# mvenouziou/Boosted_DETR

Hardware: AMD Instinct MI355X
Metric: images/sec training step (fwd+matcher+loss+bwd), 640x640 N=100 (higher is better)
Workload: dtype f32 (conv/GEMM products as 3 split-f16 [fwd] / split-bf16 [grad] MFMA products, f32 accumulate)

## Files before the change

### boosted_detr_amd/csrc/p16.hip

```cpp
#include "p16.h"

namespace {

__global__ __launch_bounds__(256) void p16_pack_kernel(const float* __restrict__ x, int64_t n8, void* __restrict__ f16_out, void* __restrict__ bf16_out,
                                                       int* __restrict__ overflow_flag, float f16_scale) {
    for (int64_t i = (int64_t)blockIdx.x * blockDim.x + threadIdx.x; i < n8; i += (int64_t)gridDim.x * blockDim.x) {
        const f32x4 a = reinterpret_cast<const f32x4*>(x)[2 * i], b = reinterpret_cast<const f32x4*>(x)[2 * i + 1];
        const float v[8] = {a[0], a[1], a[2], a[3], b[0], b[1], b[2], b[3]};
        if (f16_out) {
            const float vs[8] = {v[0] * f16_scale, v[1] * f16_scale, v[2] * f16_scale, v[3] * f16_scale, v[4] * f16_scale, v[5] * f16_scale, v[6] * f16_scale, v[7] * f16_scale};
            p16_store8<true>(reinterpret_cast<char*>(f16_out) + i * 32, vs);
            if (overflow_flag && p16_f16_overflow(vs)) *overflow_flag = 1;
        }
        if (bf16_out) p16_store8<false>(reinterpret_cast<char*>(bf16_out) + i * 32, v);
    }
}

template <bool F16>
__global__ __launch_bounds__(256) void p16_unpack_kernel(const void* __restrict__ p, int64_t n8, float* __restrict__ out) {
    for (int64_t i = (int64_t)blockIdx.x * blockDim.x + threadIdx.x; i < n8; i += (int64_t)gridDim.x * blockDim.x) {
        float v[8];
        p16_load8<F16>(reinterpret_cast<const char*>(p) + i * 32, v);
        reinterpret_cast<f32x4*>(out)[2 * i] = f32x4{v[0], v[1], v[2], v[3]};
        reinterpret_cast<f32x4*>(out)[2 * i + 1] = f32x4{v[4], v[5], v[6], v[7]};
    }
}

__global__ __launch_bounds__(256) void p16_pack_wt_kernel(const float* __restrict__ w, int K, int R, int S, int C, void* __restrict__ wt) {
    const int64_t total = (int64_t)(K / 8) * R * S * C;
    for (int64_t i = (int64_t)blockIdx.x * blockDim.x + threadIdx.x; i < total; i += (int64_t)gridDim.x * blockDim.x) {
        const int c = (int)(i % C); int64_t t = i / C;
        const int tap = (int)(t % (R * S)); const int kg = (int)(t / (R * S));
        const int r = tap / S, s = tap - r * S;
        const int src_tap = (R - 1 - r) * S + (S - 1 - s);
        float v[8];
#pragma unroll
        for (int e = 0; e < 8; ++e) v[e] = w[((int64_t)(kg * 8 + e) * R * S + src_tap) * C + c];
        p16_store8<false>(reinterpret_cast<char*>(wt) + (((int64_t)c * R * S + tap) * K + kg * 8) * 4, v);
    }
}

template <bool NT>
__global__ __launch_bounds__(256) void p16_pack_weights_multi_kernel(const int64_t* __restrict__ table, int* __restrict__ overflow_flag) {
    const int64_t* row = table + (int64_t)blockIdx.y * 7;
    const float* w = reinterpret_cast<const float*>(row[0]);
    char* wf = reinterpret_cast<char*>(row[1]);
    char* wt = reinterpret_cast<char*>(row[2]);
    const int K = (int)row[3], R = (int)row[4], S = (int)row[5], C = (int)row[6];
    const int64_t n8 = (int64_t)K * R * S * C / 8;
    for (int64_t i = (int64_t)blockIdx.x * blockDim.x + threadIdx.x; i < n8; i += (int64_t)gridDim.x * blockDim.x) {
        if (wf != nullptr) {
            const f32x4 a = ld_stream4<NT>(w, 2 * i), b = ld_stream4<NT>(w, 2 * i + 1);
            const float v[8] = {a[0] * P16_W_SCALE, a[1] * P16_W_SCALE, a[2] * P16_W_SCALE, a[3] * P16_W_SCALE,
                                b[0] * P16_W_SCALE, b[1] * P16_W_SCALE, b[2] * P16_W_SCALE, b[3] * P16_W_SCALE};
            p16_store8<true>(wf + i * 32, v);
            if (overflow_flag && p16_f16_overflow(v)) *overflow_flag = 1;
        }
        if (wt != nullptr) {
            const int c = (int)(i % C); int64_t t = i / C;
            const int tap = (int)(t % (R * S)); const int kg = (int)(t / (R * S));
            const int r = tap / S, s2 = tap - r * S;
            const int src_tap = (R - 1 - r) * S + (S - 1 - s2);
            float v[8];
#pragma unroll
            for (int e = 0; e < 8; ++e) v[e] = ld_stream<NT>(w + ((int64_t)(kg * 8 + e) * R * S + src_tap) * C + c);
            p16_store8<false>(wt + (((int64_t)c * R * S + tap) * K + kg * 8) * 4, v);
        }
    }
}

}

extern "C" int bdetr_p16_pack_conv_weights_multi(const int64_t* table, int ntensors, int* overflow_flag, void* stream) {
    BDETR_CHECK_ARG(table && ntensors > 0, "bdetr_p16_pack_conv_weights_multi: bad arguments");
    STREAM_DISPATCH(stream_on(STREAM_OPTIM), NT,
                    hipLaunchKernelGGL(p16_pack_weights_multi_kernel<NT>, dim3(48, ntensors), dim3(256), 0, (hipStream_t)stream, table, overflow_flag));
    return bdetr_launch_status("p16_pack_conv_weights_multi");
}

extern "C" int bdetr_p16_pack(const float* x, int64_t n, void* f16_out, void* bf16_out, int* overflow_flag, void* stream) {
    BDETR_CHECK_ARG(x && n > 0 && n % 8 == 0 && (f16_out || bf16_out), "bdetr_p16_pack: bad arguments (n %% 8 == 0 required)");
    hipLaunchKernelGGL(p16_pack_kernel, dim3(ew_grid(n / 8, 256, 2)), dim3(256), 0, (hipStream_t)stream, x, n / 8, f16_out, bf16_out, overflow_flag, 1.f);
    return bdetr_launch_status("p16_pack");
}

extern "C" int bdetr_p16_unpack(const void* p, int is_f16, int64_t n, float* out, void* stream) {
    BDETR_CHECK_ARG(p && out && n > 0 && n % 8 == 0, "bdetr_p16_unpack: bad arguments (n %% 8 == 0 required)");
    if (is_f16) hipLaunchKernelGGL((p16_unpack_kernel<true>), dim3(ew_grid(n / 8, 256, 2)), dim3(256), 0, (hipStream_t)stream, p, n / 8, out);
    else        hipLaunchKernelGGL((p16_unpack_kernel<false>), dim3(ew_grid(n / 8, 256, 2)), dim3(256), 0, (hipStream_t)stream, p, n / 8, out);
    return bdetr_launch_status("p16_unpack");
}

extern "C" int bdetr_p16_pack_conv_weights(const float* w, int K, int R, int S, int C, void* w_f16, void* wt_bf16, int* overflow_flag, void* stream) {
    BDETR_CHECK_ARG(w && K > 0 && R > 0 && S > 0 && C > 0 && K % 8 == 0 && C % 8 == 0, "bdetr_p16_pack_conv_weights: K and C must be multiples of 8");
    hipStream_t st = (hipStream_t)stream;
    const int64_t n = (int64_t)K * R * S * C;
    if (w_f16) hipLaunchKernelGGL(p16_pack_kernel, dim3(ew_grid(n / 8, 256, 2)), dim3(256), 0, st, w, n / 8, w_f16, (void*)nullptr, overflow_flag, P16_W_SCALE);
    if (wt_bf16) hipLaunchKernelGGL(p16_pack_wt_kernel, dim3(ew_grid(n / 8, 256, 1)), dim3(256), 0, st, w, K, R, S, C, wt_bf16);
    return bdetr_launch_status("p16_pack_conv_weights");
}

namespace {
__global__ __launch_bounds__(256) void s2d_pack_bf16_kernel(const float* __restrict__ x, int N, int H, int W, void* __restrict__ out) {
    const int H2 = H >> 1, W2 = W >> 1;
    const int64_t n = (int64_t)N * H2 * W2 * 2;
    for (int64_t t = (int64_t)blockIdx.x * blockDim.x + threadIdx.x; t < n; t += (int64_t)gridDim.x * blockDim.x) {
        const int a = (int)(t & 1); int64_t p = t >> 1;
        const int j = (int)(p % W2); p /= W2; const int i = (int)(p % H2); const int b_ = (int)(p / H2);
        const f32x4* row = reinterpret_cast<const f32x4*>(x) + ((int64_t)b_ * H + 2 * i + a) * W + 2 * j;
        const f32x4 p0 = row[0], p1 = row[1];
        const float v[8] = {p0[0], p0[1], p0[2], p0[3], p1[0], p1[1], p1[2], p1[3]};
        p16_store8<false>(reinterpret_cast<char*>(out) + t * 32, v);
    }
}
__global__ __launch_bounds__(256) void s2d_unpack_dw_kernel(const float* __restrict__ dw2, float* __restrict__ dw, int K) {
    const int n = K * 7 * 7 * 4;
    for (int t = blockIdx.x * blockDim.x + threadIdx.x; t < n; t += gridDim.x * blockDim.x) {
        const int c = t & 3; int q = t >> 2;
        const int s = q % 7; q /= 7; const int r = q % 7; const int k = q / 7;
        const int rp = (r + 1) >> 1, a = (r + 1) & 1, sp = (s + 1) >> 1, b = (s + 1) & 1;
        dw[t] = dw2[k * 256 + (rp * 4 + sp) * 16 + (a * 2 + b) * 4 + c];
    }
}
}

extern "C" int bdetr_p16_s2d_pack_bf16(const float* x, int N, int H, int W, void* out_bf16, void* stream) {
    BDETR_CHECK_ARG(x && out_bf16 && N > 0 && H > 0 && W > 0 && H % 2 == 0 && W % 2 == 0, "bdetr_p16_s2d_pack_bf16: a [N,H,W,4] image with even H and W");
    const int64_t n = (int64_t)N * (H / 2) * (W / 2) * 2;
    hipLaunchKernelGGL(s2d_pack_bf16_kernel, dim3(ew_grid(n, 256, 2)), dim3(256), 0, (hipStream_t)stream, x, N, H, W, out_bf16);
    return bdetr_launch_status("p16_s2d_pack_bf16");
}
extern "C" int bdetr_p16_s2d_unpack_dw(const float* dw2, float* dw, int K, void* stream) {
    BDETR_CHECK_ARG(dw2 && dw && K > 0, "bdetr_p16_s2d_unpack_dw: bad arguments");
    hipLaunchKernelGGL(s2d_unpack_dw_kernel, dim3((K * 196 + 255) / 256), dim3(256), 0, (hipStream_t)stream, dw2, dw, K);
    return bdetr_launch_status("p16_s2d_unpack_dw");
}
```

Measured before the change: 653.0.

## Tile multi-tensor weight packing with LDS transpose and flattened work units

Rewrites the batched conv-weight pack kernel so each block handles 64x64 (K,C) tiles per tap. The source weights are read once with coalesced vector loads and reused for both the scaled f16 copy and the transposed, tap-flipped bf16 copy. The transpose goes through a swizzled shared-memory tile instead of strided scalar gathers. Work from all tensors is flattened into one 1D grid via a prefix sum over per-tensor tile counts, which replaces the fixed 48-block-per-tensor 2D grid that left small tensors underusing it and large ones undersubscribed. This adds block barriers and per-unit index search.

```diff
diff --git a/boosted_detr_amd/csrc/p16.hip b/boosted_detr_amd/csrc/p16.hip
--- a/boosted_detr_amd/csrc/p16.hip
+++ b/boosted_detr_amd/csrc/p16.hip
@@ -1,4 +1,5 @@
 #include "p16.h"
+#include "p16_pack_index.h"
 
 namespace {
 
@@ -40,31 +41,75 @@
     }
 }
 
+constexpr int PACK_MAX_ROWS = 256;
+constexpr int PACK_GRID = 256 * 8;
+
 template <bool NT>
-__global__ __launch_bounds__(256) void p16_pack_weights_multi_kernel(const int64_t* __restrict__ table, int* __restrict__ overflow_flag) {
-    const int64_t* row = table + (int64_t)blockIdx.y * 7;
-    const float* w = reinterpret_cast<const float*>(row[0]);
-    char* wf = reinterpret_cast<char*>(row[1]);
-    char* wt = reinterpret_cast<char*>(row[2]);
-    const int K = (int)row[3], R = (int)row[4], S = (int)row[5], C = (int)row[6];
-    const int64_t n8 = (int64_t)K * R * S * C / 8;
-    for (int64_t i = (int64_t)blockIdx.x * blockDim.x + threadIdx.x; i < n8; i += (int64_t)gridDim.x * blockDim.x) {
-        if (wf != nullptr) {
-            const f32x4 a = ld_stream4<NT>(w, 2 * i), b = ld_stream4<NT>(w, 2 * i + 1);
-            const float v[8] = {a[0] * P16_W_SCALE, a[1] * P16_W_SCALE, a[2] * P16_W_SCALE, a[3] * P16_W_SCALE,
-                                b[0] * P16_W_SCALE, b[1] * P16_W_SCALE, b[2] * P16_W_SCALE, b[3] * P16_W_SCALE};
-            p16_store8<true>(wf + i * 32, v);
-            if (overflow_flag && p16_f16_overflow(v)) *overflow_flag = 1;
+__global__ __launch_bounds__(256) void p16_pack_weights_multi_kernel(const int64_t* __restrict__ table, int ntensors, int* __restrict__ overflow_flag) {
+    constexpr int TK = P16_PACK_TK, TC = P16_PACK_TC;
+    static_assert(TK == 64 && TC == 64, "the lane maps below are written for 64 x 64 tiles and 256 threads");
+    __shared__ int64_t ends[PACK_MAX_ROWS];
+    __shared__ __attribute__((aligned(16))) float tile[TK * TC];
+    const int tid = threadIdx.x;
+    if (tid < ntensors) {
+        const int64_t* row = table + (int64_t)tid * 7;
+        ends[tid] = p16_pack_units(row[3], row[4], row[5], row[6]);
+    }
+    __syncthreads();
+    for (int d = 1; d < ntensors; d <<= 1) {
+        const int64_t below = (tid >= d && tid < ntensors) ? ends[tid - d] : 0;
+        __syncthreads();
+        if (tid < ntensors) ends[tid] += below;
+        __syncthreads();
+    }
+    const int64_t total = ends[ntensors - 1];
+    const int lane8 = tid & 7, line = tid >> 3;
+    int t = 0;
+    for (int64_t g = blockIdx.x; g < total; g += gridDim.x) {
+        t = p16_pack_row_of(ends, ntensors, g, t);
+        const int64_t* row = table + (int64_t)t * 7;
+        const float* w = reinterpret_cast<const float*>(row[0]);
+        char* wf = reinterpret_cast<char*>(row[1]);
+        char* wt = reinterpret_cast<char*>(row[2]);
+        const int K = (int)row[3], R = (int)row[4], S = (int)row[5], C = (int)row[6];
+        const P16PackUnit u = p16_pack_unit(g - (t > 0 ? ends[t - 1] : 0), K, C);
+        if (wf == nullptr && wt == nullptr) continue;
+        const int c = u.c0 + lane8 * 8;
+#pragma unroll
+        for (int j = 0; j < TK / 32; ++j) {
+            const int kl = line + 32 * j, k = u.k0 + kl;
+            if (k < K && c < C) {
+                const int64_t i = (((int64_t)k * R * S + u.tap) * C + c) / 8;
+                const f32x4 a = ld_stream4<NT>(w, 2 * i), b = ld_stream4<NT>(w, 2 * i + 1);
+                if (wf != nullptr) {
+                    const float v[8] = {a[0] * P16_W_SCALE, a[1] * P16_W_SCALE, a[2] * P16_W_SCALE, a[3] * P16_W_SCALE,
+                                        b[0] * P16_W_SCALE, b[1] * P16_W_SCALE, b[2] * P16_W_SCALE, b[3] * P16_W_SCALE};
+                    p16_store8<true>(wf + i * 32, v);
+                    if (overflow_flag && p16_f16_overflow(v)) *overflow_flag = 1;
+                }
+                if (wt != nullptr) {
+                    const int sw = ((kl >> 3) & 7) << 2;
+                    *reinterpret_cast<f32x4*>(&tile[kl * TC + ((lane8 * 8) ^ sw)]) = a;
+                    *reinterpret_cast<f32x4*>(&tile[kl * TC + ((lane8 * 8 + 4) ^ sw)]) = b;
+                }
+            }
         }
         if (wt != nullptr) {
-            const int c = (int)(i % C); int64_t t = i / C;
-            const int tap = (int)(t % (R * S)); const int kg = (int)(t / (R * S));
-            const int r = tap / S, s2 = tap - r * S;
-            const int src_tap = (R - 1 - r) * S + (S - 1 - s2);
-            float v[8];
+            __syncthreads();
+            const int r = u.tap / S, s2 = u.tap - r * S;
+            const int dst_tap = (R - 1 - r) * S + (S - 1 - s2);
+            const int k = u.k0 + lane8 * 8, sw = lane8 << 2;
 #pragma unroll
-            for (int e = 0; e < 8; ++e) v[e] = ld_stream<NT>(w + ((int64_t)(kg * 8 + e) * R * S + src_tap) * C + c);
-            p16_store8<false>(wt + (((int64_t)c * R * S + tap) * K + kg * 8) * 4, v);
+            for (int j = 0; j < TC / 32; ++j) {
+                const int cl = line + 32 * j, cc = u.c0 + cl;
+                if (k < K && cc < C) {
+                    float v[8];
+#pragma unroll
+                    for (int e = 0; e < 8; ++e) v[e] = tile[(lane8 * 8 + e) * TC + (cl ^ sw)];
+                    p16_store8<false>(wt + (((int64_t)cc * R * S + dst_tap) * K + k) * 4, v);
+                }
+            }
+            __syncthreads();
         }
     }
 }
@@ -73,8 +118,12 @@
 
 extern "C" int bdetr_p16_pack_conv_weights_multi(const int64_t* table, int ntensors, int* overflow_flag, void* stream) {
     BDETR_CHECK_ARG(table && ntensors > 0, "bdetr_p16_pack_conv_weights_multi: bad arguments");
-    STREAM_DISPATCH(stream_on(STREAM_OPTIM), NT,
-                    hipLaunchKernelGGL(p16_pack_weights_multi_kernel<NT>, dim3(48, ntensors), dim3(256), 0, (hipStream_t)stream, table, overflow_flag));
+    for (int t0 = 0; t0 < ntensors; t0 += PACK_MAX_ROWS) {
+        const int n = ntensors - t0 < PACK_MAX_ROWS ? ntensors - t0 : PACK_MAX_ROWS;
+        STREAM_DISPATCH(stream_on(STREAM_OPTIM), NT,
+                        hipLaunchKernelGGL(p16_pack_weights_multi_kernel<NT>, dim3(PACK_GRID), dim3(256), 0, (hipStream_t)stream, table + (int64_t)t0 * 7, n,
+                                           overflow_flag));
+    }
     return bdetr_launch_status("p16_pack_conv_weights_multi");
 }
 
diff --git a/boosted_detr_amd/csrc/p16_pack_index.h b/boosted_detr_amd/csrc/p16_pack_index.h
--- /dev/null
+++ b/boosted_detr_amd/csrc/p16_pack_index.h
@@ -0,0 +1,29 @@
+#pragma once
+#include <stdint.h>
+
+#if defined(__HIPCC__)
+#define P16_PACK_HD __host__ __device__
+#else
+#define P16_PACK_HD
+#endif
+
+constexpr int P16_PACK_TK = 64, P16_PACK_TC = 64;
+
+struct P16PackUnit { int tap, k0, c0; };
+
+P16_PACK_HD inline int64_t p16_pack_units(int64_t K, int64_t R, int64_t S, int64_t C) {
+    return R * S * ((K + P16_PACK_TK - 1) / P16_PACK_TK) * ((C + P16_PACK_TC - 1) / P16_PACK_TC);
+}
+P16_PACK_HD inline P16PackUnit p16_pack_unit(int64_t u, int K, int C) {
+    const int ct = (C + P16_PACK_TC - 1) / P16_PACK_TC, kt = (K + P16_PACK_TK - 1) / P16_PACK_TK;
+    P16PackUnit r;
+    r.c0 = (int)(u % ct) * P16_PACK_TC; u /= ct;
+    r.k0 = (int)(u % kt) * P16_PACK_TK;
+    r.tap = (int)(u / kt);
+    return r;
+}
+P16_PACK_HD inline int p16_pack_row_of(const int64_t* ends, int n, int64_t g, int from) {
+    int t = from;
+    while (t < n - 1 && g >= ends[t]) ++t;
+    return t;
+}
```

After: 657.7, median of 6. About the same (+0.7%).
